# wolearyc/ramannoodle

Measured on AMD Instinct MI355X. Metric: structures/sec (GNN polarizability eval), higher is better.
Workload: dtype f32

## Files before the change

### ramannoodle_amd/csrc/api.hip

```cpp
#include <hip/hip_runtime.h>

#include <cmath>
#include <cstring>
#include <memory>
#include <mutex>
#include <string>
#include <vector>

#include "forward.hpp"

using namespace rn;

static std::string g_create_error;
std::string &rn_potgnn::create_error() { return g_create_error; }

namespace rn {
const char *const kKernelNames[K_COUNT] = {
    "geom_rbf", "node_init", "proj_node", "proj_edge_c1", "node_agg", "proj_edge_c3",
    "proj_c2", "edge_agg", "readout_mlp", "readout_reduce", "c2_pairs"};
}

namespace {


// ... 203 lines not shown
  h->cfg = *cfg;
  std::memcpy(h->lattice, lattice, sizeof(h->lattice));
  std::memcpy(h->mean, mean, sizeof(h->mean));
  std::memcpy(h->stdv, stddev, sizeof(h->stdv));
  h->snap_pairs = getenv("RN_POTGNN_KEEP_STAGES") && atoi(getenv("RN_POTGNN_KEEP_STAGES")) == 2;
  h->keep_stages = getenv("RN_POTGNN_KEEP_STAGES") && atoi(getenv("RN_POTGNN_KEEP_STAGES")) != 0 && !h->snap_pairs;
  h->debug_sync = getenv("RN_POTGNN_DEBUG_SYNC") && atoi(getenv("RN_POTGNN_DEBUG_SYNC")) != 0;
  if (const char *e = getenv("RN_POTGNN_INTERLEAVE")) h->interleave = atoi(e) != 0;
  if (const char *e = getenv("RN_POTGNN_MFMA")) h->mfma_f16_requested = !(e[0] == 'f' && e[1] == '3');
  h->mfma_f16 = h->mfma_f16_requested;
  if (const char *e = getenv("RN_POTGNN_TAPE_FUSED")) h->tape_fused = atoi(e) != 0;
  if (const char *e = getenv("RN_POTGNN_TAPE_PS")) h->tape_ps = atoi(e) != 0;
  h->split_projections = getenv("RN_POTGNN_SPLIT_PROJ") ? atoi(getenv("RN_POTGNN_SPLIT_PROJ")) != 0 : true;
  h->want_pair_rows = !(getenv("RN_POTGNN_PAIR_ROWS") && atoi(getenv("RN_POTGNN_PAIR_ROWS")) == 0);
  h->want_c2_pairs = !(getenv("RN_POTGNN_C2_PAIRS") && atoi(getenv("RN_POTGNN_C2_PAIRS")) == 0);

  const PlanKnobs knobs = read_plan_knobs();
  h->d = plan_dims(*cfg, knobs);
  h->plan = plan_graph(*cfg, h->d, edge_a, edge_b, atom_types, cus, knobs);

  rn_potgnn *hp = h.get();
  rc = guarded<rn_potgnn>(nullptr, [&]() {
    HIP_TRY(hipSetDevice(cfg->device));
    hp->g = upload(hp->plan, hp->g_ints);
    double ms[18];
    std::memcpy(ms, hp->mean, sizeof(hp->mean));
    std::memcpy(ms + 9, hp->stdv, sizeof(hp->stdv));
    hp->d_mean_std.ensure(sizeof(ms));
    HIP_TRY(hipMemcpy(hp->d_mean_std.p, ms, sizeof(ms), hipMemcpyHostToDevice));
    hp->lay = layout_weights(hp->cfg, hp->d);
// ... 643 lines not shown
    HIP_TRY(hipMemcpy(lat.p, lattice, 9 * sizeof(double), hipMemcpyHostToDevice));
    HIP_TRY(hipMemcpy(pos.p, positions, n * 3 * sizeof(double), hipMemcpyHostToDevice));
    launch_radius_graph(lat.as<double>(), pos.as<double>(), num_atoms, (float)cutoff,
                        adj.as<unsigned char>(), nullptr);
    HIP_TRY(hipGetLastError());
    HIP_TRY(hipDeviceSynchronize());
    HIP_TRY(hipMemcpy(adjacency, adj.p, n * n, hipMemcpyDeviceToHost));
  });
}

int rn_potgnn_config_flags(const rn_potgnn *h) {
  if (!h) return -1;
  std::lock_guard<std::recursive_mutex> hold(h->lock);
  const RunChoices c = choose(h, true, false);
  return (c.fused ? 1 : 0) | (c.folded_gate ? 2 : 0) | (c.split_f16 ? 4 : 0) | (c.narrow ? 8 : 0) | (c.range_fallback ? 16 : 0) |
         (c.every_pass_role_split ? 256 : 0) | (c.node_atom ? 512 : 0) | (c.pair_rows ? 1024 : 0) | (c.c2_pairs ? 2048 : 0);
}

int rn_potgnn_debug_ps_schedule(const int32_t *rb, const int32_t *re, int32_t num_destinations, int32_t back, int32_t ring_tiles,
                                int32_t *window) {
  if (!rb || !re || num_destinations < 0 || back < 1 || back > 8 || ring_tiles < 1 || ring_tiles > 64) return RN_ERR_INVALID_ARGUMENT;
  int w = 0;
  const bool ok = edge_ps_tile_ok(rb, re, num_destinations, back, ring_tiles, &w);
  if (window) *window = w;
  return ok ? 1 : 0;
}

int64_t rn_potgnn_num_triplets(const rn_potgnn *h) { return h ? h->g.T : -1; }

int rn_potgnn_debug_triplets(rn_potgnn *h, int32_t *idx_i, int32_t *idx_j, int32_t *idx_k,
                             int32_t *slot5, int32_t *slot6) {
// ... 56 lines not shown
```

### ramannoodle_amd/csrc/forward.hip

```cpp
#include <hip/hip_runtime.h>

#include <algorithm>
#include <chrono>
#include <cstdio>
#include <cstdlib>
#include <cstring>
#include <thread>
#include <vector>

#include "forward.hpp"

namespace rn {

template <typename T>
int chunk_frames(const rn_potgnn *h) {
  if (sizeof(T) == 4) return h->chunk;
  const size_t budget = std::max(h->f64_budget, (size_t)h->chunk * per_structure_elems(h, lean_workspace(h)) * sizeof(float));
  const size_t per64 = per_structure_elems(h, false) * sizeof(double);
  return (int)std::max<size_t>(1, std::min<size_t>((size_t)h->chunk, budget / std::max<size_t>(per64, 1)));
}

bool lean_workspace(const rn_potgnn *h) {
  return (h->plan.use_fused && h->plan.use_node_fused && h->plan.use_readout_fused) || h->plan.use_narrow;
}
// ... 166 lines not shown
    const T gauss = (T)h->cfg.gauss_coefficient;
    if constexpr (sizeof(T) == 4) {
      if (io.pos32) {
        if (ch.pair_rows) launch_geom_rbf_pairs_pos32(io.pos32, S, h->g, lat, lat_stride, P.offsets, gauss, h->d, unit4, edge[0], st());
        else launch_geom_rbf_pos32(io.pos32, S, h->g, lat, lat_stride, P.offsets, gauss, h->d, unit4, edge[0], st(), ch.narrow);
        done = true;
      } else if (ch.pair_rows) {
        launch_geom_rbf_pairs(io.pos, S, h->g, lat, lat_stride, P.offsets, gauss, h->d, unit4, edge[0], st());
        done = true;
      }
    }
    if (!done) launch_geom_rbf<T>(io.pos, S, h->g, lat, lat_stride, P.offsets, gauss, h->d, unit4, edge[0], st(), ch.narrow);
    h->last_in_order = ch.narrow;
    h->last_pair_rows = ch.pair_rows;
  }
  {
    Timer t(h, st(), K_NODE_INIT);
    launch_node_init<T>(P.node_table, S, h->g, h->d, node[0], io.types, st());
  }
  cur = 0;
  snapshot(0);
}

template <typename T>
void ChunkRun<T>::run_stages() {
  begin();
  for (int p = 0; p < h->cfg.num_message_passes; ++p) {
    stage_project(p);
    stage_aggregate(p);
  }
}

template <typename T>
void ChunkRun<T>::project(const T *X, int64_t R, int K, const T *WT, int NOUT, T *Y, const T *bias, int amode, const T *nd) {
  if constexpr (sizeof(T) == 4) {
    if (h->mfma_f16 && h->split_projections &&
// ... 5 lines not shown

template <typename T>
void ChunkRun<T>::stage_project(int p) {
  const PassW<T> &w = prec<T>(h).pass[p];
  const Graph &g = h->g;
  const Dims d = h->d;
  const int nxt = cur ^ 1;
  target_tape(p + 1, nxt);
  if constexpr (sizeof(T) == 4) {
    if (ch.narrow) {
      Timer t(h, st(), K_NODE_AGG);
      launch_node_narrow(edge[cur], node[cur], node[nxt], S, g, d, w, st());
      return;
    }
  }
  {
    Timer t(h, st(), K_PROJ_NODE);
    if (ch.node_centred) project(node[cur], MN, d.FnP, w.c1_WnT_c, 2 * d.FnP, npc1, w.c1_bias_c, 0, nullptr);
    else project(node[cur], MN, d.FnP, w.c1_WnT, 2 * d.FnP, npc1, w.c1_bias, 0, nullptr);
  }
  bool node_fused = false;
  if constexpr (sizeof(T) == 4) {
    if (ch.fused && h->plan.use_node_fused) {
      Timer t(h, st(), K_NODE_AGG);
      if (ch.node_atom) launch_node_atom(edge[cur], node[cur], npc1, node[nxt], S, g, d, w, st(), ch.pair_rows);
      else launch_node_fused(edge[cur], node[cur], npc1, node[nxt], S, g, d, w, h->mfma_f16, ch.node_centred, st());
      node_fused = true;
    }
  }
  if (!node_fused) {
    {
      Timer t(h, st(), K_PROJ_EDGE_C1);
      project(edge[cur], ME, d.FeP, w.c1_WeT, 2 * d.FnP, bufA, nullptr, 0, nullptr);
    }
    {
      Timer t(h, st(), K_NODE_AGG);
      launch_node_agg<T>(npc1, bufA, node[cur], node[nxt], S, g, d, w, st());
    }
  }
  {
// ... 81 lines not shown
      const double *ms = h->d_mean_std.as<double>();
      launch_readout_narrow(edge[cur], unit4, S, g, d, P.ro, ms, ms + 9, io.vec6, io.alpha, io.alpha_raw,
                            h->keep_stages ? bufA : nullptr, st());
      HIP_TRY(hipGetLastError());
      return;
    }
  }
  int pol_stride = 32;
  {
    Timer t(h, st(), K_READOUT_MLP);
    const int HP = std::max(d.FeP, 32);
    bool done = false;
    if constexpr (sizeof(T) == 4) {
      if (ch.fused && h->plan.use_readout_fused) {
        pol_stride = h->keep_stages ? 32 : 16;
        launch_readout_fused(edge[cur], ME, P.ro, bufA, h->mfma_f16, st(), ch.pair_rows, pol_stride);
        done = true;
      }
    }
    if (!done) {
      launch_rowgemm<T>(edge[cur], ME, d.FeP, P.ro.W0T, HP, bufA, P.ro.scale0, P.ro.shift0, true, 0,
                        nullptr, g, st());
      launch_rowgemm<T>(bufA, ME, HP, P.ro.W3T, HP, bufB, P.ones, P.ro.b3, true, 0, nullptr, g, st());
      launch_rowgemm<T>(bufB, ME, HP, P.ro.W5T, 32, bufA, nullptr, P.ro.b5, false, 0, nullptr, g,
                        st());
    }
  }
  {
    Timer t(h, st(), K_READOUT_REDUCE);
    const double *ms = h->d_mean_std.as<double>();
    launch_readout_reduce<T>(bufA, unit4, S, g, ms, ms + 9, io.vec6, io.alpha, io.alpha_raw, st(), pol_stride);
// ... 89 lines not shown
    HIP_TRY(hipStreamWaitEvent(user, lanes[l].done.get(), 0));
  }
  if (!sync) return;
  HIP_TRY(hipStreamSynchronize(user));
  if (timers) resolve_timers(h);
  check_ps_fail(h);
}

template <typename T>
void forward_device(rn_potgnn *h, const ForwardIO<T> &io, int64_t S, hipStream_t user, bool sync) {
  ensure_precision<T>(h);
  Precision<T> &P = prec<T>(h);
  const int N = h->cfg.num_atoms;
  const int lanes = h->plan.num_lanes;
  behind_caller(h, user, P.lanes, lanes);
  auto make = [&](int lane, int64_t first, int s) { return ChunkRun<T>(h, P.lanes[lane], io.at(first, N, h->d.Fe), s); };
  int64_t done = 0;
  const int capacity = chunk_frames<T>(h);
  const int64_t pieces = (S + capacity - 1) / capacity;
  const int chunk = (int)std::max<int64_t>(1, std::min<int64_t>(capacity, (S + pieces - 1) / std::max<int64_t>(pieces, 1)));
  h->train_S = 0;
  while (done < S) {
    const int64_t left = S - done;
    if (lanes == 2 && h->interleave && !h->keep_stages && !h->snap_pairs && left > 1) {
      const int64_t both = std::min<int64_t>(left, 2 * (int64_t)chunk);
      const int sa = (int)((both + 1) / 2), sb = (int)(both - sa);
      ChunkRun<T> a = make(0, done, sa), b = make(1, done + sa, sb);
      run_pair<T>(h, a, b);
      h->last_chunk_structs = sa;
      done += both;
    } else {
// ... 266 lines not shown
```

### ramannoodle_amd/csrc/forward.hpp

```cpp
#pragma once
#include "handle.hpp"

namespace rn {

bool lean_workspace(const rn_potgnn *h);
size_t per_structure_elems(const rn_potgnn *h, bool lean);
size_t bufA_width(const rn_potgnn *h, bool lean);
template <typename T>
int chunk_frames(const rn_potgnn *h);
void size_chunk(rn_potgnn *h);
void refresh_mfma_mode(rn_potgnn *h);
template <typename T>
void refresh_pass_flags(rn_potgnn *h);
template <typename T>
void device_setup(rn_potgnn *h, T *w, hipStream_t st);
template <typename T>
void upload_weights(rn_potgnn *h);
template <typename T>
void ensure_precision(rn_potgnn *h);

template <typename T>
T *stage(DeviceBuf &buf, const void *host, size_t bytes) {
  buf.ensure(bytes);
  HIP_TRY(hipMemcpy(buf.p, host, bytes, hipMemcpyHostToDevice));
// ... 33 lines not shown
    o.desc = from(desc, Fe);
    return o;
  }
};

template <typename T>
struct ChunkRun {
  rn_potgnn *h;
  Lane<T> *ln;
  ForwardIO<T> io;
  int S;
  RunChoices ch;
  int cur = 0;
  T *node[2], *edge[2], *unit4, *npc1, *np3, *bufA, *bufB;
  int64_t MN, ME;

  ChunkRun(rn_potgnn *h_, Lane<T> &l, const ForwardIO<T> &io_, int S_);
  hipStream_t st() const { return ln->stream.get(); }
  void target_tape(int slot, int which);
  void snapshot(int p);
  void begin();
  void run_stages();
  void project(const T *X, int64_t R, int K, const T *WT, int NOUT, T *Y, const T *bias, int amode, const T *nd);
  void stage_project(int p);
  void stage_aggregate(int p);
  void edge_unfused_in_blocks(int p);
  void finish();
  T *tape_agg(int p);
};

void check_ps_fail(rn_potgnn *h);
template <typename T>
void behind_caller(rn_potgnn *h, hipStream_t user, Lane<T> *lanes, int n);
// ... 60 lines not shown
```

### ramannoodle_amd/csrc/fused_common.hpp

```cpp
#pragma once
#include "device_utils.hpp"
#include "kernels.hpp"

namespace rn {

typedef float f32x4 __attribute__((ext_vector_type(4)));
typedef float f32x2 __attribute__((ext_vector_type(2)));

#ifndef RN_FUSED_PK
#define RN_FUSED_PK 1
#endif
#ifndef RN_FUSED_PRIO
#define RN_FUSED_PRIO 3
#endif
#ifndef RN_FUSED_PRIO_LATE
#define RN_FUSED_PRIO_LATE 0
#endif
#ifndef RN_NODE_PRIO
#define RN_NODE_PRIO 3
#endif
#ifndef RN_FUSED_NK_SAMEROUND
#define RN_FUSED_NK_SAMEROUND 0
#endif
#ifndef RN_E3_PAIRWISE
// ... 272 lines not shown
  for (int j = 0; j < 4; ++j)
#pragma unroll
    for (int i = 0; i < 4; ++i) af[4 * j + i] = u[j][i];
}
}

struct NodeFusedArgs {
  const float *edge;
  const float *node_in;
  const float *npc1;
  float *node_out;
  int S;
  Graph g;
  Dims d;
  PassW<float> w;
};

namespace {
constexpr int LDG = FP + 4;
struct NodeFusedLds {
  size_t bufP, atile, gated, nj, lnp, ints, total;
};
__host__ __device__ inline NodeFusedLds node_fused_lds(int maxD, int maxN) {
  auto up = [](size_t b) { return (b + 15) & ~size_t(15); };
  NodeFusedLds L;
  size_t off = 0;
  L.bufP = off; off += up((size_t)NG * LDQ * 4);
  L.atile = off; off += (size_t)NG * FP * 4;
  L.gated = off; off += up((size_t)maxD * LDG * 4);
  L.nj = off; off += up((size_t)maxN * 2 * FP * 4);
// ... 9 lines not shown
```

### ramannoodle_amd/csrc/handle.hpp

```cpp
#pragma once
#include <cstdint>
#include <string>
#include <vector>

#include "graph_plan.hpp"
#include "host_runtime.hpp"
#include "increments.hpp"
#include "kernels.hpp"
#include "weight_layout.hpp"

namespace rn {

enum KernelId {
  K_GEOM = 0, K_NODE_INIT, K_PROJ_NODE, K_PROJ_EDGE_C1, K_NODE_AGG, K_PROJ_EDGE_C3, K_PROJ_C2,
  K_EDGE_AGG, K_READOUT_MLP, K_READOUT_REDUCE, K_C2_PAIRS, K_COUNT
};
extern const char *const kKernelNames[K_COUNT];

template <typename T>
struct Lane {
  Stream stream;
  Event done;
  DeviceBuf unit4, node[2], edge[2], npc1, np3, bufA, bufB;
  DeviceBuf fbA, fbB;
};

template <typename T>
struct Precision {
  bool ready = false;
  DeviceBuf weights;
  DeviceBuf lattice;
  std::vector<PassW<T>> pass;
  ReadoutW<T> ro{};
  const T *offsets = nullptr, *node_table = nullptr, *ones = nullptr;
  Lane<T> lanes[2];
  std::vector<DeviceBuf> snap_node, snap_edge;
  std::vector<DeviceBuf> tape_node, tape_edge, tape_agg;
  DeviceBuf bw[18];
  Stream side;
// ... 15 lines not shown

struct rn_potgnn {
  mutable std::recursive_mutex lock;
  rn_potgnn_config cfg{};
  rn::Dims d{};
  int chunk = 1;
  size_t f64_budget = 0;
  bool keep_stages = false;
  bool snap_pairs = false;
  bool last_pair_rows = false;
  bool debug_sync = false;
  rn::GraphPlan plan;
  bool split_projections = true;
  bool want_pair_rows = true;
  bool want_c2_pairs = true;
  rn::DeviceBuf step_seg, step_stage;
  rn::PinnedBuf step_host;
  bool tape_ps = true;
  bool mfma_f16 = true;
  bool mfma_f16_requested = true;
  bool mfma_range_fallback = false;
  rn::Graph g{};
  rn::DeviceBuf g_ints;
  rn::DeviceBuf ps_fail;
  double lattice[9], mean[9], stdv[9];
  rn::DeviceBuf d_mean_std;
  std::vector<float> packed;
  rn::PackedLayout lay;
  rn::Precision<float> f32;
  rn::Precision<double> f64;
// ... 115 lines not shown
```

### ramannoodle_amd/csrc/kernels.hpp

```cpp
#pragma once
#include <hip/hip_runtime.h>
#include <algorithm>
#include <cstddef>
#include <cstdint>
#include <vector>

namespace rn {

struct Graph {
  int N, E;
  const int *edge_a;
  const int *edge_b;
  const int *out_ptr;
  const int *in_ptr;
  const int *in_edge;
  const int *in_pos;
  const int *atom_type;
  const int *rev_edge;
  int NP;
  const int *pair_of_edge;
  const int *pair_a, *pair_b;
  int num_tiles;
  const int *tile_begin;
  int max_tile_out_rows;
// ... 288 lines not shown
  const double *F, *FT, *ref, *alpha_ref, *xs, *coef, *scale;
  const int *poff;
  int64_t K3;
  int J, order, Pmax;
};
void launch_interp_alpha(const double *pos, int64_t S, const InterpModel &m, double *alpha, hipStream_t st);
void launch_interp_jacobian(const double *pos, int64_t S, const InterpModel &m, double *g, double *jac, hipStream_t st);

constexpr size_t kFusedLdsBudget = 80 * 1024;
size_t edge_fused_lds_bytes(const Graph &g);
size_t edge_fused_lds_bytes(int tile_out_rows, int tile_in_rows, int tile_nodes);
bool edge_fused_supported(const Graph &g, Dims d);
size_t node_fused_lds_bytes(const Graph &g);
size_t node_fused_lds_bytes(int tile_in_rows, int tile_nodes);
void launch_readout_fused(const float *edge, int64_t M, const ReadoutW<float> &w, float *pol, bool f16,
                          hipStream_t st, bool pair_rows = false, int pol_stride = 32 );
size_t node_atom_lds_bytes(int max_deg);
void launch_node_atom(const float *edge, const float *node_in, const float *npc1, float *node_out, int S, const Graph &g,
                      Dims d, const PassW<float> &w, hipStream_t st, bool pair_rows = false);
void launch_node_fused(const float *edge, const float *node_in, const float *npc1, float *node_out, int S,
                       const Graph &g, Dims d, const PassW<float> &w, bool f16, bool centred, hipStream_t st);
size_t edge_ps_lds_bytes(int tile_out_rows, int tile_in_rows, bool gram);
int edge_ps_ring_tiles(bool gram);
int edge_ps_gram_window();
bool edge_ps_tile_ok(const int *rb, const int *re, int D, int back, int ring, int *window);
void launch_edge_ps(const float *edge_in, float *edge_out, const float *node, const float *np3, float *agg_out, int S,
                    const Graph &g, Dims d, const PassW<float> &w, int *fail, hipStream_t st, bool pair_rows = false,
                    bool f16 = true ,
                    const float *c2_rows = nullptr );
bool edge_ps_takes_c2_rows(const Graph &g, bool pair_rows, bool f16);

void launch_c2_pairs(const float *node, float *out, int S, const Graph &g, Dims d, const PassW<float> &w, hipStream_t st);

struct DerivedOp {
// ... 27 lines not shown
```

### ramannoodle_amd/csrc/kernels_fused.hip

```cpp
#include "fused_common.hpp"

namespace rn {


#ifndef RN_NODE_REGRING
#define RN_NODE_REGRING 2
#endif
#ifndef RN_NODE_PROBE
#define RN_NODE_PROBE 0
#endif
template <bool PAD, bool F16, bool ZM = false >
__global__ __launch_bounds__(256, 4) void node_block_fused_kernel(NodeFusedArgs a) {
  extern __shared__ __attribute__((aligned(16))) unsigned char smem_raw[];
  const Graph &g = a.g;
  const NodeFusedLds L = node_fused_lds(g.nt_max_in_rows, g.nt_max_nodes);
  float *bufP = reinterpret_cast<float *>(smem_raw + L.bufP);
  float *atile = reinterpret_cast<float *>(smem_raw + L.atile);
  float *gated = reinterpret_cast<float *>(smem_raw + L.gated);
  float *nj = reinterpret_cast<float *>(smem_raw + L.nj);
  float *lnp = reinterpret_cast<float *>(smem_raw + L.lnp);
  float *s_c1g = lnp, *s_c1b = lnp + 2 * FP, *s_fg = lnp + 4 * FP, *s_fb = lnp + 5 * FP;
  int *d_edge = reinterpret_cast<int *>(smem_raw + L.ints), *d_bl = d_edge + g.nt_max_in_rows;

  const int tid = threadIdx.x, lane = tid & 63;
// ... 156 lines not shown
      const Vec4<float> old = load4<float>(a.node_in + (nrow0 + j0 + n) * FP + c0);
      Vec4<float> out;
#pragma unroll
      for (int k = 0; k < 4; ++k) out.v[k] = fast_tanh(old.v[k] + ln.v[k]);
      store4(a.node_out + (nrow0 + j0 + n) * FP + c0, out);
    }
  }
}

size_t node_fused_lds_bytes(const Graph &g) { return node_fused_lds(g.nt_max_in_rows, g.nt_max_nodes).total; }
size_t node_fused_lds_bytes(int tile_in_rows, int tile_nodes) { return node_fused_lds(tile_in_rows, tile_nodes).total; }

void launch_node_fused(const float *edge, const float *node_in, const float *npc1, float *node_out, int S,
                       const Graph &g, Dims d, const PassW<float> &w, bool f16, bool centred, hipStream_t st) {
  if (S == 0 || g.N == 0) return;
  NodeFusedArgs a{edge, node_in, npc1, node_out, S, g, d, w};
  const bool pad = d.Fn != d.FnP;
  const size_t lds = node_fused_lds_bytes(g);
  auto kern = f16 ? (centred ? (pad ? &node_block_fused_kernel<true, true, true> : &node_block_fused_kernel<false, true, true>)
                             : (pad ? &node_block_fused_kernel<true, true> : &node_block_fused_kernel<false, true>))
                  : (pad ? &node_block_fused_kernel<true, false> : &node_block_fused_kernel<false, false>);
  if (lds > 48 * 1024)
    (void)hipFuncSetAttribute(reinterpret_cast<const void *>(kern), hipFuncAttributeMaxDynamicSharedMemorySize,
                              (int)lds);
  static int cus = 0;
  if (cus == 0) {
    int dev = 0;
    hipDeviceProp_t prop;
    if (hipGetDevice(&dev) == hipSuccess && hipGetDeviceProperties(&prop, dev) == hipSuccess)
      cus = prop.multiProcessorCount;
    if (cus <= 0) cus = 256;
  }
  int per_cu = 0;
  if (hipOccupancyMaxActiveBlocksPerMultiprocessor(&per_cu, kern, 256, lds) != hipSuccess || per_cu < 1) per_cu = 1;
  per_cu = std::min(per_cu, 4);
  int nsg = per_cu * cus / g.nt_num;
  nsg = nsg < 1 ? 1 : (nsg > S ? S : nsg);
  kern<<<(unsigned)nsg * (unsigned)g.nt_num, 256, lds, st>>>(a);
}

struct ReadoutFusedArgs {
  const float *edge;
  float *pol;
  int64_t M;
  ReadoutW<float> w;
  int pol_stride;
};

template <bool F16, bool PRE = false, int NW = (F16 ? 8 : 4)>
__global__ __launch_bounds__(64 * NW, 2) void readout_fused_kernel(ReadoutFusedArgs a, int tiles_per_wave) {
  constexpr int LDW = FP + 4;
  constexpr int LDH = FP + 8;
  constexpr int kW64 = F16 ? 2 * FP * LDH * 2 : FP * LDW * 4, kW16 = F16 ? 2 * 16 * LDH * 2 : 16 * LDW * 4;
  extern __shared__ __attribute__((aligned(16))) unsigned char ro_smem[];
  unsigned char *w0_raw = ro_smem, *w3_raw = w0_raw + kW64, *w5_raw = w3_raw + kW64;
  float *slab_all = reinterpret_cast<float *>(w5_raw + kW16);
  float *s_scale0 = slab_all + NW * 16 * LDW, *s_shift0 = s_scale0 + FP, *s_b3 = s_shift0 + FP, *s_b5 = s_b3 + FP;
  const int tid = threadIdx.x, lane = tid & 63, wave = tid >> 6;
  const int l15 = lane & 15, quad = lane >> 4;
  auto put = [&](unsigned char *raw, int rows, int n, int k, float v) {
    if constexpr (F16) {
      _Float16 *h = reinterpret_cast<_Float16 *>(raw), *l = h + rows * LDH;
      const _Float16 hi = (_Float16)v;
      h[n * LDH + k] = hi;
      l[n * LDH + k] = (_Float16)(v - (float)hi);
    } else {
      reinterpret_cast<float *>(raw)[n * LDW + k] = v;
    }
  };
  const float ps0 = F16 ? a.w.mfma_scale[0] : 1.0f, inv0 = F16 ? a.w.mfma_scale[1] : 1.0f;
  const float ps3 = F16 ? a.w.mfma_scale[2] : 1.0f, inv3 = F16 ? a.w.mfma_scale[3] : 1.0f;
  const float ps5 = F16 ? a.w.mfma_scale[4] : 1.0f, inv5 = F16 ? a.w.mfma_scale[5] : 1.0f;
  for (int i = tid; i < FP * FP; i += 64 * NW) {
    const int k = i / FP, n = i % FP;
    put(w0_raw, FP, n, k, ps0 * a.w.W0T[i]);
    put(w3_raw, FP, n, k, ps3 * a.w.W3T[i]);
  }
  for (int i = tid; i < FP * 16; i += 64 * NW) {
    const int k = i / 16, n = i % 16;
    put(w5_raw, 16, n, k, ps5 * a.w.W5T[k * 32 + n]);
  }
  if (tid < FP) {
    s_scale0[tid] = a.w.scale0[tid] * inv0;
    s_shift0[tid] = a.w.shift0[tid];
    s_b3[tid] = a.w.b3[tid];
    if (tid < 16) s_b5[tid] = a.w.b5[tid];
  }
  __syncthreads();
  float *slab = slab_all + wave * 16 * LDW;
  const int64_t num_tiles = (a.M + 15) / 16;
  const int64_t first = ((int64_t)blockIdx.x * NW + wave) * tiles_per_wave;

  f16x8 ah[2], al[2];
  auto operand = [&](const float (&af)[KS]) {
    if constexpr (F16) {
      split_f16x8(af, ah[0], al[0]);
      split_f16x8(af + 8, ah[1], al[1]);
    }
  };
  auto operand_pairs = [&](const float (&af)[KS]) {
    union { float f[4]; f16x8 h; } u[4];
#pragma unroll
    for (int j = 0; j < 4; ++j)
#pragma unroll
      for (int i = 0; i < 4; ++i) u[j].f[i] = af[4 * j + i];
    ah[0] = u[0].h; al[0] = u[1].h; ah[1] = u[2].h; al[1] = u[3].h;
// ... 26 lines not shown
      af[4 * j] = v.x; af[4 * j + 1] = v.y; af[4 * j + 2] = v.z; af[4 * j + 3] = v.w;
    }
  };

  float nxt[KS];
  auto fetch = [&](int64_t tile) {
    int64_t row = tile * 16 + l15;
    if (row >= a.M) row = a.M - 1;
    const float *p = a.edge + row * FP + quad * KS;
#pragma unroll
    for (int j = 0; j < 4; ++j) {
      const float4 v = *reinterpret_cast<const float4 *>(p + 4 * j);
      nxt[4 * j] = v.x; nxt[4 * j + 1] = v.y; nxt[4 * j + 2] = v.z; nxt[4 * j + 3] = v.w;
    }
  };
  if (first < num_tiles) fetch(first);
  for (int it = 0; it < tiles_per_wave; ++it) {
    const int64_t tile = first + it;
    if (tile >= num_tiles) break;
    float af[KS];
#pragma unroll
    for (int k = 0; k < KS; ++k) af[k] = nxt[k];
    if (it + 1 < tiles_per_wave && tile + 1 < num_tiles) fetch(tile + 1);
    f32x4 acc;
    if constexpr (PRE) operand_pairs(af);
    else operand(af);
#pragma unroll
    for (int nt = 0; nt < 4; ++nt) {
      product(af, w0_raw, FP, nt, acc);
      const int col = nt * 16 + l15;
#pragma unroll
      for (int rr = 0; rr < 4; ++rr)
        slab[(4 * quad + rr) * LDW + col] = ssp_fast(acc[rr] * s_scale0[col] + s_shift0[col]);
    }
    load_slab(af);
    operand(af);
#pragma unroll
    for (int nt = 0; nt < 4; ++nt) {
// ... 2 lines not shown
#pragma unroll
      for (int rr = 0; rr < 4; ++rr) slab[(4 * quad + rr) * LDW + col] = ssp_fast(fmaf(acc[rr], inv3, s_b3[col]));
    }
    load_slab(af);
    operand(af);
    product(af, w5_raw, 16, 0, acc);
#pragma unroll
    for (int rr = 0; rr < 4; ++rr) {
      const int64_t row = tile * 16 + 4 * quad + rr;
      if (row < a.M) a.pol[row * a.pol_stride + l15] = fmaf(acc[rr], inv5, s_b5[l15]);
    }
  }
}

void launch_readout_fused(const float *edge, int64_t M, const ReadoutW<float> &w, float *pol, bool f16,
                          hipStream_t st, bool pair_rows, int pol_stride) {
  if (M == 0) return;
  ReadoutFusedArgs a{edge, pol, M, w, pol_stride};
  const int64_t tiles = (M + 15) / 16;
  const int tpw = 8;
  auto launch = [&](auto kern, int nw, bool f16w) {
    constexpr int LDW = FP + 4, LDH = FP + 8;
    const size_t lds = (f16w ? (size_t)2 * (2 * FP * LDH * 2) + 2 * 16 * LDH * 2 : (size_t)2 * FP * LDW * 4 + 16 * LDW * 4) +
                       (size_t)nw * 16 * LDW * 4 + (3 * FP + 16) * 4;
    if (lds > 48 * 1024)
      (void)hipFuncSetAttribute(reinterpret_cast<const void *>(kern), hipFuncAttributeMaxDynamicSharedMemorySize, (int)lds);
    const unsigned blocks = (unsigned)((tiles + (int64_t)nw * tpw - 1) / ((int64_t)nw * tpw));
    kern<<<blocks, 64 * nw, lds, st>>>(a, tpw);
  };
  if (f16 && pair_rows) launch(&readout_fused_kernel<true, true>, 8, true);
  else if (f16) launch(&readout_fused_kernel<true>, 8, true);
  else launch(&readout_fused_kernel<false>, 4, false);
}

size_t edge_fused_lds_bytes(const Graph &g) {
  return fused_lds(g.max_tile_out_rows, g.max_tile_in_rows, g.max_tile_nodes).total;
}
size_t edge_fused_lds_bytes(int rows, int in_rows, int nodes) { return fused_lds(rows, in_rows, nodes).total; }

bool edge_fused_supported(const Graph &g, Dims d) {
  return d.FnP == 64 && d.FeP == 64 && g.E > 0 && edge_fused_lds_bytes(g) <= kFusedLdsBudget;
}

}
```

### ramannoodle_amd/csrc/kernels_node_atom.hip

```cpp
#include "fused_common.hpp"
#include <type_traits>

namespace rn {
namespace {
constexpr int NA_D = 4;
static_assert((NA_D & (NA_D - 1)) == 0, "ring slots are addressed with a mask");

struct NodeAtomLds {
  size_t atile, land, part, lnp, tab, total;
};
__host__ __device__ inline NodeAtomLds node_atom_lds(int max_deg) {
  auto up = [](size_t b) { return (b + 15) & ~size_t(15); };
  NodeAtomLds L;
  size_t off = 0;
  L.atile = off; off += (size_t)NA_D * NG * FP * 4;
  L.land = off; off += (size_t)4 * 256 * 16;
  L.part = off; off += (size_t)4 * NG * 4 * 4;
  L.lnp = off; off += (size_t)2 * FP * 4;
  L.tab = off; off += up(((size_t)NG * (size_t)(max_deg > 0 ? max_deg : 1) + NG) * 4);
  L.total = off;
  return L;
}

#ifndef RN_NA_PROBE
// ... 62 lines not shown
  for (int k = 0; k < 4; ++k) {
    gfm[k] = -kLog2e * a.w.c1_norm.g[fcol + k];
    bfm[k] = -kLog2e * a.w.c1_norm.b[fcol + k];
    gcm[k] = 2.0f * kLog2e * a.w.c1_norm.g[FP + fcol + k];
    bcm[k] = 2.0f * kLog2e * a.w.c1_norm.b[FP + fcol + k];
  }
  const float kClamp = 15.0f * 2.0f * kLog2e;
  const int nvalid = min(max(a.d.Fn - fcol, 0), 4);
  const float inv2n = 1.0f / (float)(2 * a.d.Fn), invn = 1.0f / (float)a.d.Fn;
  const float eps_s = 1e-5f * s1 * s1;
  __syncthreads();
  if (sg >= a.S) return;
  const int nframes = (a.S - sg + nsg - 1) / nsg;

  const int arow = j0 + min(l15, natoms - 1);
  auto seed_ptr = [&](int f, int t) { return a.npc1 + ((int64_t)(sg + f * nsg) * g.N + arow) * (2 * FP) + t * FP + fcol; };
  auto old_ptr = [&](int f) { return a.node_in + ((int64_t)(sg + f * nsg) * g.N + arow) * FP + fcol; };
  f32x4 seed[2];
  {
    const float4 s0 = *reinterpret_cast<const float4 *>(seed_ptr(0, 0)), s1v = *reinterpret_cast<const float4 *>(seed_ptr(0, 1));
    seed[0] = f32x4{s0.x, s0.y, s0.z, s0.w} * s1;
    seed[1] = f32x4{s1v.x, s1v.y, s1v.z, s1v.w} * s1;
    asm volatile("" : "+v"(seed[0]), "+v"(seed[1]));
  }
  auto request_old = [&](int f) { dma16(old_ptr(f), land + (2 + (f & 1)) * 1024 + wave * 256); };
  auto request_frame = [&](int f) {
    dma16(seed_ptr(f, 0), land + wave * 256);
    dma16(seed_ptr(f, 1), land + 1024 + wave * 256);
    request_old(f);
  };

  auto epilogue = [&](int f, const f32x4 &sum, const f32x4 *old_given) {
// ... 102 lines not shown
    return true;
  };
  static_assert(NA_D == 4, "the round loop is unrolled over a four-slot ring");
  for (;;) {
    if (!round(std::integral_constant<int, 0>{})) break;
    if (!round(std::integral_constant<int, 1>{})) break;
    if (!round(std::integral_constant<int, 2>{})) break;
    if (!round(std::integral_constant<int, 3>{})) break;
  }
  asm volatile("s_waitcnt vmcnt(0)" ::: "memory");
}

size_t node_atom_lds_bytes(int max_deg) { return node_atom_lds(max_deg).total; }

void launch_node_atom(const float *edge, const float *node_in, const float *npc1, float *node_out, int S, const Graph &g,
                      Dims d, const PassW<float> &w, hipStream_t st, bool pair_rows) {
  if (S == 0 || g.N == 0) return;
  NodeFusedArgs a{edge, node_in, npc1, node_out, S, g, d, w};
  const bool pad = d.Fn != d.FnP;
  const size_t lds = node_atom_lds_bytes(g.na_max_deg);
  auto kern = pair_rows ? (pad ? &node_block_atom_kernel<true, true> : &node_block_atom_kernel<false, true>)
                        : (pad ? &node_block_atom_kernel<true, false> : &node_block_atom_kernel<false, false>);
  if (lds > 48 * 1024)
    (void)hipFuncSetAttribute(reinterpret_cast<const void *>(kern), hipFuncAttributeMaxDynamicSharedMemorySize, (int)lds);
  static int cus = 0;
  if (cus == 0) {
    int dev = 0;
    hipDeviceProp_t prop;
    if (hipGetDevice(&dev) == hipSuccess && hipGetDeviceProperties(&prop, dev) == hipSuccess) cus = prop.multiProcessorCount;
    if (cus <= 0) cus = 256;
  }
  int per_cu = 0;
  if (hipOccupancyMaxActiveBlocksPerMultiprocessor(&per_cu, kern, 256, lds) != hipSuccess || per_cu < 1) per_cu = 1;
// ... 8 lines not shown
```

### ramannoodle_amd/csrc/reverse.hip

```cpp
#include <hip/hip_runtime.h>

#include <algorithm>
#include <cstdlib>
#include <vector>

#include "forward.hpp"

namespace rn {

enum { DE0, DE1, DN0, DN1, DNX, DPQ, DNP3, DC2, DPROD, DBC1, DNPC1, DPOL, DUNIT, DH, POL, DOUT, DPROD2, BWN };

template <typename T>
void reverse_pass(rn_potgnn *h, ChunkRun<T> &c, const Reverse<T> &rv) {
  Precision<T> &P = prec<T>(h);
  const PackedLayout &L = h->lay;
  const Graph &g = h->g;
  const Dims d = h->d;
  const int N = g.N, E = g.E, NP = h->cfg.num_message_passes;
  const int S = rv.S, B = rv.B, C = S * B;
  const int HP = std::max(d.FeP, 32);
  hipStream_t st = c.st();
  const size_t ce = (size_t)C * E, cn = (size_t)C * N, fe = (size_t)S * E, fn = (size_t)S * N;
  const size_t sizes[BWN] = {ce * d.FeP, ce * d.FeP, cn * d.FnP, cn * d.FnP, cn * d.FnP,
                             ce * 4 * d.FeP, cn * 6 * d.FeP, ce * std::max(2 * d.FeP, HP), ce * d.FnP,
// ... 163 lines not shown
  for (int p = 0; p <= NP; ++p) {
    P.tape_node[p].ensure((size_t)S * h->g.N * h->d.FnP * sizeof(T));
    P.tape_edge[p].ensure((size_t)S * h->g.E * h->d.FeP * sizeof(T));
    P.tape_agg[p].ensure((size_t)S * h->g.E * h->d.FeP * sizeof(T));
  }
  Lane<T> &ln = P.lanes[0];
  ln.bufA.ensure((size_t)S * h->g.E * bufA_width(h, false) * sizeof(T));
  ln.bufB.ensure((size_t)S * h->g.E * 4 * h->d.FeP * sizeof(T));
}

template <typename T>
ChunkRun<T> taped_forward(rn_potgnn *h, const ForwardIO<T> &io , int S) {
  Precision<T> &P = prec<T>(h);
  ensure_tape<T>(h, S);
  P.tape_on = true;
  ChunkRun<T> c(h, P.lanes[0], io, S);
  try {
    c.run_stages();
  } catch (...) {
    P.tape_on = false;
    throw;
  }
  P.tape_on = false;
  return c;
}

template <typename T>
void jacobian(rn_potgnn *h, const double *host_pos, double *host_jac ) {
  ensure_precision<T>(h);
  const int N = h->g.N;
// ... 215 lines not shown
```

### ramannoodle_amd/pmodel/potgnn.py

```python
from __future__ import annotations

import ctypes as C
from collections import OrderedDict

import numpy as np
import torch
from numpy.typing import NDArray
from torch.autograd.function import once_differentiable

from ramannoodle_amd import _lib
from ramannoodle_amd.abstract import PolarizabilityModel
from ramannoodle_amd.constants import RAMAN_TENSOR_CENTRAL_DIFFERENCE
from ramannoodle_amd.exceptions import verify_ndarray_shape
from ramannoodle_amd.pmodel import graph as graph_utils
from ramannoodle_amd.pmodel._device import (DeviceIncrements, _ptr, check_out as _check_out, device_frames, device_out,
                                            mode_arrays, raman_arguments)

_VEC_TO_TENSOR = np.array([[0, 3, 4], [3, 1, 5], [4, 5, 2]])


def polarizability_vectors_to_tensors(vectors):
    if vectors.ndim != 2 or vectors.shape[1] != 6:
        raise ValueError(f"polarizability_vectors has wrong size: {list(vectors.shape)} != [_,6]")
    return vectors[:, _VEC_TO_TENSOR]
# ... 906 lines not shown
        lib = _lib.load()
        cap = 64 * 1024 * 1024
        buf = np.empty(cap, dtype=np.float32)
        rows, cols = C.c_int64(), C.c_int64()
        rc = lib.rn_potgnn_debug_stage(handle, stage, index, _ptr(buf), cap, C.byref(rows),
                                       C.byref(cols))
        _lib.check(rc, handle, "rn_potgnn_debug_stage")
        return buf[: rows.value * cols.value].reshape(rows.value, cols.value).copy()

    def config_flags(self) -> dict:
        flags = _lib.load().rn_potgnn_config_flags(self._ensure_handle())
        return {"fused_edge_block": bool(flags & 1), "folded_gate_scale": bool(flags & 2),
                "split_f16_mfma": bool(flags & 4), "narrow_kernels": bool(flags & 8),
                "mfma_range_fallback": bool(flags & 16),
                "role_split_edge_block": bool(flags & 256), "atom_owning_node_block": bool(flags & 512),
                "split_f16_pair_rows": bool(flags & 1024), "c2_per_atom_pair": bool(flags & 2048)}

    def set_profiling(self, mode: int) -> None:
        self._profiling = int(mode)
        if self._handle is not None:
            _lib.load().rn_potgnn_set_profiling(self._handle, self._profiling)

    def kernel_times(self) -> dict:
        handle = self._ensure_handle()
        lib = _lib.load()
        names = (C.c_char_p * 16)()
        ms = (C.c_double * 16)()
        launches = (C.c_int64 * 16)()
        n = lib.rn_potgnn_kernel_times(handle, names, ms, launches, 16)
        return {names[i].decode(): (ms[i], launches[i]) for i in range(max(n, 0))}

# ... 112 lines not shown
```

Baseline: 66250.

## Precompute per-call pass-0 node tables and stream prebuilt readout weight image

When node features at pass 0 depend only on atom type and not on the frame, the node init and pass-0 node projection now run once per call over N atoms. The node-atom kernel reads those tables with a zero frame stride instead of per-frame copies. Separately, a one-time kernel prebuilds the split-f16 readout weight image in LDS layout. The fused readout then copies it with 16-byte loads and runs a persistent grid sized to about 2x CU count with grid-stride tiles, replacing per-block weight conversion. This adds extra small kernel launches per call and assumes pass-0 inputs are frame-invariant.

```diff
diff --git a/ramannoodle_amd/csrc/api.hip b/ramannoodle_amd/csrc/api.hip
--- a/ramannoodle_amd/csrc/api.hip
+++ b/ramannoodle_amd/csrc/api.hip
@@ -1,5 +1,6 @@
 #include <hip/hip_runtime.h>
 
+#include <algorithm>
 #include <cmath>
 #include <cstring>
 #include <memory>
@@ -241,6 +242,9 @@
   h->split_projections = getenv("RN_POTGNN_SPLIT_PROJ") ? atoi(getenv("RN_POTGNN_SPLIT_PROJ")) != 0 : true;
   h->want_pair_rows = !(getenv("RN_POTGNN_PAIR_ROWS") && atoi(getenv("RN_POTGNN_PAIR_ROWS")) == 0);
   h->want_c2_pairs = !(getenv("RN_POTGNN_C2_PAIRS") && atoi(getenv("RN_POTGNN_C2_PAIRS")) == 0);
+  h->want_pass0_tables = !(getenv("RN_POTGNN_PASS0_TABLES") && atoi(getenv("RN_POTGNN_PASS0_TABLES")) == 0);
+  h->want_readout_stream = !(getenv("RN_POTGNN_READOUT_STREAM") && atoi(getenv("RN_POTGNN_READOUT_STREAM")) == 0);
+  if (const char *e = getenv("RN_POTGNN_READOUT_WGS")) h->readout_wgs = std::max(0, atoi(e));
 
   const PlanKnobs knobs = read_plan_knobs();
   h->d = plan_dims(*cfg, knobs);
@@ -914,7 +918,8 @@
   std::lock_guard<std::recursive_mutex> hold(h->lock);
   const RunChoices c = choose(h, true, false);
   return (c.fused ? 1 : 0) | (c.folded_gate ? 2 : 0) | (c.split_f16 ? 4 : 0) | (c.narrow ? 8 : 0) | (c.range_fallback ? 16 : 0) |
-         (c.every_pass_role_split ? 256 : 0) | (c.node_atom ? 512 : 0) | (c.pair_rows ? 1024 : 0) | (c.c2_pairs ? 2048 : 0);
+         (c.every_pass_role_split ? 256 : 0) | (c.node_atom ? 512 : 0) | (c.pair_rows ? 1024 : 0) | (c.c2_pairs ? 2048 : 0) |
+         (h->last_pass0_tables ? 4096 : 0);
 }
 
 int rn_potgnn_debug_ps_schedule(const int32_t *rb, const int32_t *re, int32_t num_destinations, int32_t back, int32_t ring_tiles,
diff --git a/ramannoodle_amd/csrc/forward.hip b/ramannoodle_amd/csrc/forward.hip
--- a/ramannoodle_amd/csrc/forward.hip
+++ b/ramannoodle_amd/csrc/forward.hip
@@ -204,12 +204,40 @@
     h->last_in_order = ch.narrow;
     h->last_pair_rows = ch.pair_rows;
   }
-  {
+  if (!pass0_tables) {
     Timer t(h, st(), K_NODE_INIT);
     launch_node_init<T>(P.node_table, S, h->g, h->d, node[0], io.types, st());
   }
   cur = 0;
   snapshot(0);
+}
+
+template <typename T>
+void ChunkRun<T>::prepare_call(bool tables, bool image) {
+  if constexpr (sizeof(T) == 4) {
+    Precision<T> &P = prec<T>(h);
+    const Graph &g = h->g;
+    const Dims d = h->d;
+    if (tables) {
+      const PassW<T> &w = P.pass[0];
+      ln->node0.ensure((size_t)g.N * d.FnP * sizeof(T));
+      ln->npc1_0.ensure((size_t)g.N * 2 * d.FnP * sizeof(T));
+      {
+        Timer t(h, st(), K_NODE_INIT);
+        launch_node_init<T>(P.node_table, 1, g, d, ln->node0.template as<T>(), nullptr, st());
+      }
+      {
+        Timer t(h, st(), K_PROJ_NODE);
+        project(ln->node0.template as<T>(), g.N, d.FnP, w.c1_WnT_c, 2 * d.FnP, ln->npc1_0.template as<T>(), w.c1_bias_c, 0, nullptr);
+      }
+    }
+    if (image) {
+      Timer t(h, st(), K_READOUT_MLP);
+      ln->ro_image.ensure(readout_image_bytes());
+      launch_readout_image(P.ro, ln->ro_image.template as<unsigned char>(), st());
+    }
+    HIP_TRY(hipGetLastError());
+  }
 }
 
 template <typename T>
@@ -245,7 +273,8 @@
       return;
     }
   }
-  {
+  const bool tables = pass0_tables && p == 0;
+  if (!tables) {
     Timer t(h, st(), K_PROJ_NODE);
     if (ch.node_centred) project(node[cur], MN, d.FnP, w.c1_WnT_c, 2 * d.FnP, npc1, w.c1_bias_c, 0, nullptr);
     else project(node[cur], MN, d.FnP, w.c1_WnT, 2 * d.FnP, npc1, w.c1_bias, 0, nullptr);
@@ -254,7 +283,9 @@
   if constexpr (sizeof(T) == 4) {
     if (ch.fused && h->plan.use_node_fused) {
       Timer t(h, st(), K_NODE_AGG);
-      if (ch.node_atom) launch_node_atom(edge[cur], node[cur], npc1, node[nxt], S, g, d, w, st(), ch.pair_rows);
+      if (ch.node_atom && tables)
+        launch_node_atom(edge[cur], ln->node0.template as<T>(), ln->npc1_0.template as<T>(), node[nxt], S, g, d, w, st(), ch.pair_rows, true);
+      else if (ch.node_atom) launch_node_atom(edge[cur], node[cur], npc1, node[nxt], S, g, d, w, st(), ch.pair_rows);
       else launch_node_fused(edge[cur], node[cur], npc1, node[nxt], S, g, d, w, h->mfma_f16, ch.node_centred, st());
       node_fused = true;
     }
@@ -366,7 +397,8 @@
     if constexpr (sizeof(T) == 4) {
       if (ch.fused && h->plan.use_readout_fused) {
         pol_stride = h->keep_stages ? 32 : 16;
-        launch_readout_fused(edge[cur], ME, P.ro, bufA, h->mfma_f16, st(), ch.pair_rows, pol_stride);
+        launch_readout_fused(edge[cur], ME, P.ro, bufA, h->mfma_f16, st(), ch.pair_rows, pol_stride,
+                             readout_stream ? ln->ro_image.template as<unsigned char>() : nullptr, h->readout_wgs);
         done = true;
       }
     }
@@ -486,7 +518,21 @@
   const int N = h->cfg.num_atoms;
   const int lanes = h->plan.num_lanes;
   behind_caller(h, user, P.lanes, lanes);
-  auto make = [&](int lane, int64_t first, int s) { return ChunkRun<T>(h, P.lanes[lane], io.at(first, N, h->d.Fe), s); };
+  bool tables = false, image = false;
+  if constexpr (sizeof(T) == 4) {
+    const RunChoices ch = choose(h, true, P.tape_on);
+    tables = h->want_pass0_tables && ch.node_atom && !ch.narrow && !io.types && !h->keep_stages && !h->snap_pairs && !P.tape_on;
+    image = h->want_readout_stream && ch.fused && !ch.narrow && h->plan.use_readout_fused && h->mfma_f16 && !h->keep_stages;
+    if (tables || image)
+      for (int l = 0; l < lanes; ++l) ChunkRun<T>(h, P.lanes[l], io, 1).prepare_call(tables, image);
+  }
+  h->last_pass0_tables = tables;
+  auto make = [&](int lane, int64_t first, int s) {
+    ChunkRun<T> c(h, P.lanes[lane], io.at(first, N, h->d.Fe), s);
+    c.pass0_tables = tables;
+    c.readout_stream = image;
+    return c;
+  };
   int64_t done = 0;
   const int capacity = chunk_frames<T>(h);
   const int64_t pieces = (S + capacity - 1) / capacity;
diff --git a/ramannoodle_amd/csrc/forward.hpp b/ramannoodle_amd/csrc/forward.hpp
--- a/ramannoodle_amd/csrc/forward.hpp
+++ b/ramannoodle_amd/csrc/forward.hpp
@@ -71,9 +71,12 @@
   int cur = 0;
   T *node[2], *edge[2], *unit4, *npc1, *np3, *bufA, *bufB;
   int64_t MN, ME;
+  bool pass0_tables = false;
+  bool readout_stream = false;
 
   ChunkRun(rn_potgnn *h_, Lane<T> &l, const ForwardIO<T> &io_, int S_);
   hipStream_t st() const { return ln->stream.get(); }
+  void prepare_call(bool tables, bool image);
   void target_tape(int slot, int which);
   void snapshot(int p);
   void begin();
diff --git a/ramannoodle_amd/csrc/fused_common.hpp b/ramannoodle_amd/csrc/fused_common.hpp
--- a/ramannoodle_amd/csrc/fused_common.hpp
+++ b/ramannoodle_amd/csrc/fused_common.hpp
@@ -310,6 +310,7 @@
   Graph g;
   Dims d;
   PassW<float> w;
+  int node_stride, npc1_stride;
 };
 
 namespace {
diff --git a/ramannoodle_amd/csrc/handle.hpp b/ramannoodle_amd/csrc/handle.hpp
--- a/ramannoodle_amd/csrc/handle.hpp
+++ b/ramannoodle_amd/csrc/handle.hpp
@@ -23,6 +23,7 @@
   Event done;
   DeviceBuf unit4, node[2], edge[2], npc1, np3, bufA, bufB;
   DeviceBuf fbA, fbB;
+  DeviceBuf node0, npc1_0, ro_image;
 };
 
 template <typename T>
@@ -68,6 +69,10 @@
   bool split_projections = true;
   bool want_pair_rows = true;
   bool want_c2_pairs = true;
+  bool want_pass0_tables = true;
+  bool last_pass0_tables = false;
+  bool want_readout_stream = true;
+  int readout_wgs = 0;
   rn::DeviceBuf step_seg, step_stage;
   rn::PinnedBuf step_host;
   bool tape_ps = true;
diff --git a/ramannoodle_amd/csrc/kernels.hpp b/ramannoodle_amd/csrc/kernels.hpp
--- a/ramannoodle_amd/csrc/kernels.hpp
+++ b/ramannoodle_amd/csrc/kernels.hpp
@@ -326,10 +326,14 @@
 size_t node_fused_lds_bytes(const Graph &g);
 size_t node_fused_lds_bytes(int tile_in_rows, int tile_nodes);
 void launch_readout_fused(const float *edge, int64_t M, const ReadoutW<float> &w, float *pol, bool f16,
-                          hipStream_t st, bool pair_rows = false, int pol_stride = 32 );
+                          hipStream_t st, bool pair_rows = false, int pol_stride = 32 ,
+                          const unsigned char *image = nullptr ,
+                          int max_wgs = 0 );
+size_t readout_image_bytes();
+void launch_readout_image(const ReadoutW<float> &w, unsigned char *image, hipStream_t st);
 size_t node_atom_lds_bytes(int max_deg);
 void launch_node_atom(const float *edge, const float *node_in, const float *npc1, float *node_out, int S, const Graph &g,
-                      Dims d, const PassW<float> &w, hipStream_t st, bool pair_rows = false);
+                      Dims d, const PassW<float> &w, hipStream_t st, bool pair_rows = false, bool per_atom_inputs = false);
 void launch_node_fused(const float *edge, const float *node_in, const float *npc1, float *node_out, int S,
                        const Graph &g, Dims d, const PassW<float> &w, bool f16, bool centred, hipStream_t st);
 size_t edge_ps_lds_bytes(int tile_out_rows, int tile_in_rows, bool gram);
diff --git a/ramannoodle_amd/csrc/kernels_fused.hip b/ramannoodle_amd/csrc/kernels_fused.hip
--- a/ramannoodle_amd/csrc/kernels_fused.hip
+++ b/ramannoodle_amd/csrc/kernels_fused.hip
@@ -194,7 +194,7 @@
 void launch_node_fused(const float *edge, const float *node_in, const float *npc1, float *node_out, int S,
                        const Graph &g, Dims d, const PassW<float> &w, bool f16, bool centred, hipStream_t st) {
   if (S == 0 || g.N == 0) return;
-  NodeFusedArgs a{edge, node_in, npc1, node_out, S, g, d, w};
+  NodeFusedArgs a{edge, node_in, npc1, node_out, S, g, d, w, g.N, g.N};
   const bool pad = d.Fn != d.FnP;
   const size_t lds = node_fused_lds_bytes(g);
   auto kern = f16 ? (centred ? (pad ? &node_block_fused_kernel<true, true, true> : &node_block_fused_kernel<false, true, true>)
@@ -225,12 +225,58 @@
   int64_t M;
   ReadoutW<float> w;
   int pol_stride;
+  const unsigned char *image;
 };
 
-template <bool F16, bool PRE = false, int NW = (F16 ? 8 : 4)>
+namespace {
+constexpr int kRoLDH = FP + 8;
+constexpr int kRoW64 = 2 * FP * kRoLDH * 2, kRoW16 = 2 * 16 * kRoLDH * 2;
+constexpr int kRoImageW = 2 * kRoW64 + kRoW16, kRoImageV = (3 * FP + 16) * 4;
+static_assert(kRoImageW % 16 == 0 && kRoImageV % 16 == 0, "the image is staged with 16-byte copies");
+__device__ __forceinline__ void ro_put_split(unsigned char *raw, int rows, int n, int k, float v) {
+  _Float16 *h = reinterpret_cast<_Float16 *>(raw), *l = h + rows * kRoLDH;
+  const _Float16 hi = (_Float16)v;
+  h[n * kRoLDH + k] = hi;
+  l[n * kRoLDH + k] = (_Float16)(v - (float)hi);
+}
+}
+
+__global__ __launch_bounds__(256) void readout_image_kernel(ReadoutW<float> w, unsigned char *image) {
+  unsigned char *w0_raw = image, *w3_raw = w0_raw + kRoW64, *w5_raw = w3_raw + kRoW64;
+  float *vec = reinterpret_cast<float *>(image + kRoImageW);
+  const int tid = blockIdx.x * 256 + threadIdx.x, nth = gridDim.x * 256;
+  const float ps0 = w.mfma_scale[0], inv0 = w.mfma_scale[1], ps3 = w.mfma_scale[2], ps5 = w.mfma_scale[4];
+  for (int i = tid; i < FP * FP; i += nth) {
+    const int k = i / FP, n = i % FP;
+    ro_put_split(w0_raw, FP, n, k, ps0 * w.W0T[i]);
+    ro_put_split(w3_raw, FP, n, k, ps3 * w.W3T[i]);
+  }
+  for (int i = tid; i < FP * 16; i += nth) {
+    const int k = i / 16, n = i % 16;
+    ro_put_split(w5_raw, 16, n, k, ps5 * w.W5T[k * 32 + n]);
+  }
+  for (int i = tid; i < (2 * (2 * FP) + 2 * 16) * (kRoLDH - FP); i += nth) {
+    const int row = i / (kRoLDH - FP), k = FP + i % (kRoLDH - FP);
+    reinterpret_cast<_Float16 *>(image)[row * kRoLDH + k] = (_Float16)0.0f;
+  }
+  if (tid < FP) {
+    vec[tid] = w.scale0[tid] * inv0;
+    vec[FP + tid] = w.shift0[tid];
+    vec[2 * FP + tid] = w.b3[tid];
+    if (tid < 16) vec[3 * FP + tid] = w.b5[tid];
+  }
+}
+
+size_t readout_image_bytes() { return (size_t)kRoImageW + kRoImageV; }
+void launch_readout_image(const ReadoutW<float> &w, unsigned char *image, hipStream_t st) {
+  readout_image_kernel<<<16, 256, 0, st>>>(w, image);
+}
+
+template <bool F16, bool PRE = false, int NW = (F16 ? 8 : 4), bool STREAM = false>
 __global__ __launch_bounds__(64 * NW, 2) void readout_fused_kernel(ReadoutFusedArgs a, int tiles_per_wave) {
+  static_assert(F16 || !STREAM, "the weight image is the split-f16 one");
   constexpr int LDW = FP + 4;
-  constexpr int LDH = FP + 8;
+  constexpr int LDH = kRoLDH;
   constexpr int kW64 = F16 ? 2 * FP * LDH * 2 : FP * LDW * 4, kW16 = F16 ? 2 * 16 * LDH * 2 : 16 * LDW * 4;
   extern __shared__ __attribute__((aligned(16))) unsigned char ro_smem[];
   unsigned char *w0_raw = ro_smem, *w3_raw = w0_raw + kW64, *w5_raw = w3_raw + kW64;
@@ -239,37 +285,42 @@
   const int tid = threadIdx.x, lane = tid & 63, wave = tid >> 6;
   const int l15 = lane & 15, quad = lane >> 4;
   auto put = [&](unsigned char *raw, int rows, int n, int k, float v) {
-    if constexpr (F16) {
-      _Float16 *h = reinterpret_cast<_Float16 *>(raw), *l = h + rows * LDH;
-      const _Float16 hi = (_Float16)v;
-      h[n * LDH + k] = hi;
-      l[n * LDH + k] = (_Float16)(v - (float)hi);
-    } else {
-      reinterpret_cast<float *>(raw)[n * LDW + k] = v;
-    }
-  };
-  const float ps0 = F16 ? a.w.mfma_scale[0] : 1.0f, inv0 = F16 ? a.w.mfma_scale[1] : 1.0f;
-  const float ps3 = F16 ? a.w.mfma_scale[2] : 1.0f, inv3 = F16 ? a.w.mfma_scale[3] : 1.0f;
-  const float ps5 = F16 ? a.w.mfma_scale[4] : 1.0f, inv5 = F16 ? a.w.mfma_scale[5] : 1.0f;
-  for (int i = tid; i < FP * FP; i += 64 * NW) {
-    const int k = i / FP, n = i % FP;
-    put(w0_raw, FP, n, k, ps0 * a.w.W0T[i]);
-    put(w3_raw, FP, n, k, ps3 * a.w.W3T[i]);
-  }
-  for (int i = tid; i < FP * 16; i += 64 * NW) {
-    const int k = i / 16, n = i % 16;
-    put(w5_raw, 16, n, k, ps5 * a.w.W5T[k * 32 + n]);
-  }
-  if (tid < FP) {
-    s_scale0[tid] = a.w.scale0[tid] * inv0;
-    s_shift0[tid] = a.w.shift0[tid];
-    s_b3[tid] = a.w.b3[tid];
-    if (tid < 16) s_b5[tid] = a.w.b5[tid];
+    if constexpr (F16) ro_put_split(raw, rows, n, k, v);
+    else reinterpret_cast<float *>(raw)[n * LDW + k] = v;
+  };
+  const float inv3 = F16 ? a.w.mfma_scale[3] : 1.0f, inv5 = F16 ? a.w.mfma_scale[5] : 1.0f;
+  if constexpr (STREAM) {
+    static_assert(kW64 == kRoW64 && kW16 == kRoW16, "the image is this kernel's LDS layout");
+    const uint4 *img = reinterpret_cast<const uint4 *>(a.image);
+    uint4 *dst_w = reinterpret_cast<uint4 *>(ro_smem), *dst_v = reinterpret_cast<uint4 *>(s_scale0);
+    for (int i = tid; i < kRoImageW / 16; i += 64 * NW) dst_w[i] = img[i];
+    for (int i = tid; i < kRoImageV / 16; i += 64 * NW) dst_v[i] = img[kRoImageW / 16 + i];
+  } else {
+    const float ps0 = F16 ? a.w.mfma_scale[0] : 1.0f, inv0 = F16 ? a.w.mfma_scale[1] : 1.0f;
+    const float ps3 = F16 ? a.w.mfma_scale[2] : 1.0f, ps5 = F16 ? a.w.mfma_scale[4] : 1.0f;
+    for (int i = tid; i < FP * FP; i += 64 * NW) {
+      const int k = i / FP, n = i % FP;
+      put(w0_raw, FP, n, k, ps0 * a.w.W0T[i]);
+      put(w3_raw, FP, n, k, ps3 * a.w.W3T[i]);
+    }
+    for (int i = tid; i < FP * 16; i += 64 * NW) {
+      const int k = i / 16, n = i % 16;
+      put(w5_raw, 16, n, k, ps5 * a.w.W5T[k * 32 + n]);
+    }
+    if (tid < FP) {
+      s_scale0[tid] = a.w.scale0[tid] * inv0;
+      s_shift0[tid] = a.w.shift0[tid];
+      s_b3[tid] = a.w.b3[tid];
+      if (tid < 16) s_b5[tid] = a.w.b5[tid];
+    }
   }
   __syncthreads();
   float *slab = slab_all + wave * 16 * LDW;
   const int64_t num_tiles = (a.M + 15) / 16;
-  const int64_t first = ((int64_t)blockIdx.x * NW + wave) * tiles_per_wave;
+  const int64_t wave_id = (int64_t)blockIdx.x * NW + wave;
+  const int64_t step = STREAM ? (int64_t)gridDim.x * NW : 1;
+  const int64_t first = STREAM ? wave_id : wave_id * tiles_per_wave;
+  const int64_t end = STREAM ? num_tiles : (first + tiles_per_wave < num_tiles ? first + tiles_per_wave : num_tiles);
 
   f16x8 ah[2], al[2];
   auto operand = [&](const float (&af)[KS]) {
@@ -326,14 +377,12 @@
       nxt[4 * j] = v.x; nxt[4 * j + 1] = v.y; nxt[4 * j + 2] = v.z; nxt[4 * j + 3] = v.w;
     }
   };
-  if (first < num_tiles) fetch(first);
-  for (int it = 0; it < tiles_per_wave; ++it) {
-    const int64_t tile = first + it;
-    if (tile >= num_tiles) break;
+  if (first < end) fetch(first);
+  for (int64_t tile = first; tile < end; tile += step) {
     float af[KS];
 #pragma unroll
     for (int k = 0; k < KS; ++k) af[k] = nxt[k];
-    if (it + 1 < tiles_per_wave && tile + 1 < num_tiles) fetch(tile + 1);
+    if (tile + step < end) fetch(tile + step);
     f32x4 acc;
     if constexpr (PRE) operand_pairs(af);
     else operand(af);
@@ -366,21 +415,35 @@
 }
 
 void launch_readout_fused(const float *edge, int64_t M, const ReadoutW<float> &w, float *pol, bool f16,
-                          hipStream_t st, bool pair_rows, int pol_stride) {
+                          hipStream_t st, bool pair_rows, int pol_stride, const unsigned char *image, int max_wgs) {
   if (M == 0) return;
-  ReadoutFusedArgs a{edge, pol, M, w, pol_stride};
+  ReadoutFusedArgs a{edge, pol, M, w, pol_stride, image};
   const int64_t tiles = (M + 15) / 16;
   const int tpw = 8;
+  const bool stream = f16 && image != nullptr;
+  static int cus = 0;
+  if (stream && cus == 0) {
+    int dev = 0;
+    hipDeviceProp_t prop;
+    if (hipGetDevice(&dev) == hipSuccess && hipGetDeviceProperties(&prop, dev) == hipSuccess) cus = prop.multiProcessorCount;
+    if (cus <= 0) cus = 256;
+  }
   auto launch = [&](auto kern, int nw, bool f16w) {
     constexpr int LDW = FP + 4, LDH = FP + 8;
     const size_t lds = (f16w ? (size_t)2 * (2 * FP * LDH * 2) + 2 * 16 * LDH * 2 : (size_t)2 * FP * LDW * 4 + 16 * LDW * 4) +
                        (size_t)nw * 16 * LDW * 4 + (3 * FP + 16) * 4;
     if (lds > 48 * 1024)
       (void)hipFuncSetAttribute(reinterpret_cast<const void *>(kern), hipFuncAttributeMaxDynamicSharedMemorySize, (int)lds);
-    const unsigned blocks = (unsigned)((tiles + (int64_t)nw * tpw - 1) / ((int64_t)nw * tpw));
-    kern<<<blocks, 64 * nw, lds, st>>>(a, tpw);
-  };
-  if (f16 && pair_rows) launch(&readout_fused_kernel<true, true>, 8, true);
+    int64_t blocks = (tiles + (int64_t)nw * tpw - 1) / ((int64_t)nw * tpw);
+    if (stream) {
+      blocks = std::min<int64_t>(2 * (int64_t)cus, (tiles + nw - 1) / nw);
+      if (max_wgs > 0) blocks = std::min<int64_t>(blocks, max_wgs);
+    }
+    kern<<<(unsigned)blocks, 64 * nw, lds, st>>>(a, tpw);
+  };
+  if (stream && pair_rows) launch(&readout_fused_kernel<true, true, 8, true>, 8, true);
+  else if (stream) launch(&readout_fused_kernel<true, false, 8, true>, 8, true);
+  else if (f16 && pair_rows) launch(&readout_fused_kernel<true, true>, 8, true);
   else if (f16) launch(&readout_fused_kernel<true>, 8, true);
   else launch(&readout_fused_kernel<false>, 4, false);
 }
diff --git a/ramannoodle_amd/csrc/kernels_node_atom.hip b/ramannoodle_amd/csrc/kernels_node_atom.hip
--- a/ramannoodle_amd/csrc/kernels_node_atom.hip
+++ b/ramannoodle_amd/csrc/kernels_node_atom.hip
@@ -100,8 +100,8 @@
   const int nframes = (a.S - sg + nsg - 1) / nsg;
 
   const int arow = j0 + min(l15, natoms - 1);
-  auto seed_ptr = [&](int f, int t) { return a.npc1 + ((int64_t)(sg + f * nsg) * g.N + arow) * (2 * FP) + t * FP + fcol; };
-  auto old_ptr = [&](int f) { return a.node_in + ((int64_t)(sg + f * nsg) * g.N + arow) * FP + fcol; };
+  auto seed_ptr = [&](int f, int t) { return a.npc1 + ((int64_t)(sg + f * nsg) * a.npc1_stride + arow) * (2 * FP) + t * FP + fcol; };
+  auto old_ptr = [&](int f) { return a.node_in + ((int64_t)(sg + f * nsg) * a.node_stride + arow) * FP + fcol; };
   f32x4 seed[2];
   {
     const float4 s0 = *reinterpret_cast<const float4 *>(seed_ptr(0, 0)), s1v = *reinterpret_cast<const float4 *>(seed_ptr(0, 1));
@@ -234,9 +234,10 @@
 size_t node_atom_lds_bytes(int max_deg) { return node_atom_lds(max_deg).total; }
 
 void launch_node_atom(const float *edge, const float *node_in, const float *npc1, float *node_out, int S, const Graph &g,
-                      Dims d, const PassW<float> &w, hipStream_t st, bool pair_rows) {
+                      Dims d, const PassW<float> &w, hipStream_t st, bool pair_rows, bool per_atom_inputs) {
   if (S == 0 || g.N == 0) return;
-  NodeFusedArgs a{edge, node_in, npc1, node_out, S, g, d, w};
+  const int stride = per_atom_inputs ? 0 : g.N;
+  NodeFusedArgs a{edge, node_in, npc1, node_out, S, g, d, w, stride, stride};
   const bool pad = d.Fn != d.FnP;
   const size_t lds = node_atom_lds_bytes(g.na_max_deg);
   auto kern = pair_rows ? (pad ? &node_block_atom_kernel<true, true> : &node_block_atom_kernel<false, true>)
diff --git a/ramannoodle_amd/csrc/reverse.hip b/ramannoodle_amd/csrc/reverse.hip
--- a/ramannoodle_amd/csrc/reverse.hip
+++ b/ramannoodle_amd/csrc/reverse.hip
@@ -201,6 +201,7 @@
   Precision<T> &P = prec<T>(h);
   ensure_tape<T>(h, S);
   P.tape_on = true;
+  h->last_pass0_tables = false;
   ChunkRun<T> c(h, P.lanes[0], io, S);
   try {
     c.run_stages();
diff --git a/ramannoodle_amd/pmodel/potgnn.py b/ramannoodle_amd/pmodel/potgnn.py
--- a/ramannoodle_amd/pmodel/potgnn.py
+++ b/ramannoodle_amd/pmodel/potgnn.py
@@ -944,7 +944,8 @@
                 "split_f16_mfma": bool(flags & 4), "narrow_kernels": bool(flags & 8),
                 "mfma_range_fallback": bool(flags & 16),
                 "role_split_edge_block": bool(flags & 256), "atom_owning_node_block": bool(flags & 512),
-                "split_f16_pair_rows": bool(flags & 1024), "c2_per_atom_pair": bool(flags & 2048)}
+                "split_f16_pair_rows": bool(flags & 1024), "c2_per_atom_pair": bool(flags & 2048),
+                "pass0_per_atom_rows": bool(flags & 4096)}
 
     def set_profiling(self, mode: int) -> None:
         self._profiling = int(mode)
```

After: 66230, median of 2. No clear change (-0.0%).
